# wns349/tensorflow-yolo

Measured on AMD Instinct MI355X. Metric: images/sec at 1/2/4/8 MI355X + post-NMS box-set match vs CPU ref, higher is better.
Workload: dtype f16; 1 GPU; v3-608-b32-fp16; network=v3, batch_per_gpu=32, global_batch=32, weights=seeded synthetic Darknet stream (random-init), streams=1

## Files before the change

### tensorflow-yolo_amd/csrc/conv_tap.hip

```cpp
#include "conv_common.h"
#include "conv_tiles.h"
#include <cstdio>
#include <type_traits>
#include <utility>

#ifndef YOLO_TAP_ASM_MFMA
#define YOLO_TAP_ASM_MFMA 1
#endif
#ifndef YOLO_TAP_W_FIRST
#define YOLO_TAP_W_FIRST 1
#endif
#ifndef YOLO_TAP_AH_ALL
#define YOLO_TAP_AH_ALL 1
#endif
#ifndef YOLO_TAP_PIL_RECOMPUTE
#define YOLO_TAP_PIL_RECOMPUTE 0
#endif
#ifndef YOLO_TAP_PIL
#define YOLO_TAP_PIL 1
#endif
#ifndef YOLO_TAP_DBG
#define YOLO_TAP_DBG 0
#endif
#ifndef YOLO_TAP_RECOMPUTE_ADDR
#define YOLO_TAP_RECOMPUTE_ADDR 1
#endif
#ifndef YOLO_TAP_LATE_FROM
#define YOLO_TAP_LATE_FROM 4
#endif
#ifndef YOLO_TAP_STAGGER
#define YOLO_TAP_STAGGER 1
#endif

namespace yolo {

namespace {

typedef __attribute__((address_space(3))) void tap_lds_void;

__device__ __forceinline__ void tap_dma16(__amdgpu_buffer_rsrc_t rsrc, unsigned char *lds_dst, uint32_t voff, uint32_t soff) {
#if defined(__HIP_DEVICE_COMPILE__)
    __builtin_amdgcn_raw_ptr_buffer_load_lds(rsrc, (tap_lds_void *)lds_dst, 16, voff, soff, 0, 0);
#else
    (void)rsrc; (void)lds_dst; (void)voff; (void)soff;
#endif
}

template <typename T>
__device__ __forceinline__ void tap_mfma(float4v &acc, const uint4v &a, const uint4v &b) {
#if YOLO_TAP_ASM_MFMA && defined(__HIP_DEVICE_COMPILE__)
    if constexpr (sizeof(T) == 2) {
        asm volatile("v_mfma_f32_16x16x32_f16 %0, %1, %2, %0" : "+v"(acc) : "v"(a), "v"(b));
        return;
    }
#endif
    acc = mma_chunk<T>(a, b, acc);
}

template <int TM, int TP>
__device__ __forceinline__ void tap_mfma_drain(float4v (&acc)[TM][TP]) {
#if YOLO_TAP_ASM_MFMA && defined(__HIP_DEVICE_COMPILE__)
    asm volatile("s_nop 15\n\ts_nop 15" : "+v"(acc[0][0]));
#pragma unroll
    for (int a = 0; a < TM; ++a)
#pragma unroll
        for (int b = 0; b < TP; ++b) asm volatile("" : "+v"(acc[a][b]));
#endif
}

template <int N>
__device__ __forceinline__ void tap_wait_vm() {
    asm volatile("s_waitcnt vmcnt(%0)" ::"n"(N) : "memory");
}

__device__ __forceinline__ int tap_swz_w(int r) { return (0x78 >> (2 * ((r >> 2) & 3))) & 3; }

constexpr int kTapStreamBiasFloats = 512;

}

template <bool F32, int WM, int WN, int TM, int TP, int PRG, int OCC, int MODE, bool SPLITK, bool FAST = false, bool FUSE2 = false>
__global__ void __launch_bounds__(WM * WN * 64, OCC) conv3x3_tap_kernel(const ConvParams p) {
    typedef typename std::conditional<F32, float, _Float16>::type T;
    constexpr bool TWO_D = MODE == 2 || MODE == 3;
    constexpr bool S2 = MODE == 4;
    constexpr int PADQ = TWO_D ? 2 : 1;
    constexpr int NW = WM * WN;
    constexpr int S = 3;
    constexpr bool STAG = YOLO_TAP_STAGGER != 0 && !F32 && !SPLITK && TM % 2 == 0 && NW == 8 && MODE == 4 && OCC == 4;
    constexpr int TMH = TM / 2;
    constexpr bool PIL = YOLO_TAP_PIL != 0 && MODE == 1 && !F32;
    constexpr int PL = (PRG * 16) / TP;
    constexpr int ROWB = 64;
    constexpr int NA = WM * TM * 16;
    constexpr int NB = WN * TP * 16;
    constexpr int JA_TOT = NA / 16;
    constexpr int JA = (JA_TOT + NW - 1) / NW;
    constexpr int PW = (TWO_D && OCC >= 6) ? 18 : 24;
    constexpr int FROW = TWO_D ? PW : 16;
    constexpr int JP = (PRG + NW - 1) / NW;
    constexpr int CH = 4 * TM;
    constexpr int A_BYTES = NA * ROWB;
    constexpr int P_BYTES = PRG * 1024;
    static_assert(NW == 8, "eight waves");
    static_assert(JA_TOT % NW == 0 || JA_TOT < NW, "weight tile must split evenly over the waves (or be smaller than them)");
    static_assert(!TWO_D || PRG * 16 >= (NB / 16 + 2) * PW, "patch buffer too small for the 2-D tile");
    if constexpr (F32 && (TP > 2 || OCC >= 6)) return;
    if constexpr (SPLITK && !(WM == 2 && WN == 4 && TM == 4 && (TP == 2 || ((TP == 4 || TP == 3) && !F32)) && MODE == 1)) return;
    if constexpr (MODE == 3 && (TP % 2 != 0 || SPLITK)) return;
    static_assert(!FAST || (!F32 && !SPLITK && MODE != 3), "the lean epilogue: fp16, whole K, plain output");
    static_assert(!S2 || JA_TOT % NW == 0, "stride 2: every wave carries weights");
    if constexpr (S2 && (F32 || SPLITK)) return;
    static_assert(!FUSE2 || (FAST && WM == 2 && WN == 4 && TM == 4 && TP == 4), "back-to-back 1x1: the 128 x 256 tiles (eight waves)");
    constexpr int LDS_BYTES = FUSE2 && kFuse2LdsBytes > S * A_BYTES + 2 * P_BYTES ? kFuse2LdsBytes : S * A_BYTES + 2 * P_BYTES;
    __shared__ __attribute__((aligned(16))) unsigned char smem[LDS_BYTES];
    unsigned char *const smemP = smem + S * A_BYTES;

    const int tid = threadIdx.x;
#ifdef YOLO_EXPERIMENT
    const unsigned long long t_start = p.trace ? wall_clock64() : 0ull;
    const unsigned long long c_start = p.trace ? (unsigned long long)clock64() : 0ull;
    if ((p.dbg & 64) && ((__builtin_amdgcn_s_getreg(0xF804) >> 16) & 1u)) __builtin_amdgcn_s_setprio(3);
    if ((p.dbg >> 8) > 0 && ((__builtin_amdgcn_s_getreg(0xF804) >> 16) & 1u)) {
        const unsigned long long until = wall_clock64() + (unsigned long long)(p.dbg >> 8) * 25ull;
        while (wall_clock64() < until) __builtin_amdgcn_s_sleep(4);
    }
#endif
    const int lane = tid & 63;
    const int wave = __builtin_amdgcn_readfirstlane(tid >> 6);
    const int wm = wave / WN, wn = wave % WN;

    const int bid = xcd_remap(blockIdx.x, p.n_blocks);
    const int mt = (int)fdiv((uint32_t)bid, p.dtiles_n);
    const int nt = bid - mt * p.n_tiles_n;
    const int n0 = nt * NA;
    const int q0 = mt * p.q_stride;
    const bool has_a = JA_TOT % NW == 0 || wave < JA_TOT;

    const __amdgpu_buffer_rsrc_t rs_in = __builtin_amdgcn_make_buffer_rsrc(const_cast<void *>(p.in), 0, p.in_bytes, 0x00020000);
    const __amdgpu_buffer_rsrc_t rs_w = __builtin_amdgcn_make_buffer_rsrc(const_cast<void *>(p.wgt), 0, p.wgt_bytes, 0x00020000);

    const int lrow = lane >> 2;
    uint32_t a_off[JA];
#pragma unroll
    for (int j = 0; j < JA; ++j) {
        const int r = (j * NW + wave) * 16 + lrow;
        const int ws = r / (TM * 16), R = r % (TM * 16);
        const int tm = R >> 4, g4 = (R >> 2) & 3, jj = R & 3;
        const int ch = ws * (TM * 16) + g4 * CH + 4 * tm + jj;
        a_off[j] = (uint32_t)(n0 + ch) * p.wrow_bytes + (uint32_t)(((lane & 3) ^ tap_swz_w(lrow)) << 4);
    }
    const int c_begin = SPLITK ? (int)blockIdx.y * p.kunits : 0;
    const int C = SPLITK ? ((c_begin + p.kunits < (p.cin_chunks >> 2)) ? c_begin + p.kunits : (p.cin_chunks >> 2)) : (p.cin_chunks >> 2);
    const int KT = 9 * C;
    auto issue_weights = [&](int tap, int c, int slot) {
        const uint32_t ka = (uint32_t)(tap * p.cin_chunks + 4 * c) * 16;
        if (has_a) {
#pragma unroll
            for (int j = 0; j < JA; ++j) tap_dma16(rs_w, smem + slot * A_BYTES + (j * NW + wave) * 1024, a_off[j], ka);
        }
    };
    constexpr bool W_FIRST = YOLO_TAP_W_FIRST != 0 && YOLO_TAP_PIL != 0 && MODE == 1 && !F32;
    if constexpr (W_FIRST) {
        issue_weights(0, c_begin, 0);
        issue_weights(1, c_begin, 1);
        __builtin_amdgcn_sched_barrier(0);
    }
    constexpr int JP_FULL = PRG - (JP - 1) * NW;
    const bool jp_full = wave < JP_FULL;
    uint32_t b_off[JP];
    const uint32_t csw_p = (uint32_t)(((lane & 3) ^ (((lrow >> 2) & 1) << 1)) << 4);
    int t2_n = 0, t2_y0 = 0, t2_x0 = 0;
    if (TWO_D) {
        t2_n = (int)fdiv((uint32_t)mt, p.dqHW);
        const int r = mt - t2_n * p.qHW;
        const int ty = (int)fdiv((uint32_t)r, p.dqW);
        t2_y0 = ty * (NB / 16);
        t2_x0 = (r - ty * p.qW) * 16;
    }
#pragma unroll
    for (int j = 0; j < JP; ++j) {
        const int g = j * NW + wave;
        bool ok;
        int n, y, x;
        if (TWO_D) {
            const int R = g * 16 + lrow;
            const int pr = R / PW, pc = R - pr * PW;
            n = t2_n; y = t2_y0 - 1 + pr; x = t2_x0 - 1 + pc;
            ok = g < PRG && pc < 18 && pr < NB / 16 + 2 && t2_n * p.HoWo < p.M && (unsigned)y < (unsigned)p.H && (unsigned)x < (unsigned)p.W;
        } else {
            int Rp = g * 16 + lrow;
            bool in_planes = true;
            if constexpr (PIL) {
                const int plane = Rp / PL, idx = Rp - plane * PL;
                in_planes = plane < TP;
                Rp = idx * TP + plane;
            }
            const int q = q0 - (p.qW + 1) + Rp;
            ok = g < PRG && in_planes && q >= 0 && q < p.Mq;
            const int qq = ok ? q : 0;
            n = (int)fdiv((uint32_t)qq, p.dqHW);
            const int r = qq - n * p.qHW;
            y = (int)fdiv((uint32_t)r, p.dqW);
            x = r - y * p.qW;
            if (S2) { ok = ok && x < p.Wo && y < p.Ho; y *= 2; x *= 2; }
            else ok = ok && x < p.W && y < p.H;
        }
        const long long e = (long long)n * p.in_img_stride + ((long long)y * p.W + x) * p.in_ld + p.in_coff;
        b_off[j] = ok ? (uint32_t)(e * (long long)sizeof(T)) + csw_p : YOLO_INVALID_OFF;
    }

    auto issue_patch = [&](int c, int buf, uint32_t plane_off = 0u) {
        const uint32_t koff = (uint32_t)c * ROWB + plane_off;
#pragma unroll
        for (int j = 0; j < JP; ++j)
            if (j + 1 < JP || jp_full) tap_dma16(rs_in, smemP + buf * P_BYTES + (j * NW + wave) * 1024, b_off[j], koff);
    };

    float4v acc[TM][TP];
    float4v acc2[F32 ? TM : 1][F32 ? TP : 1];
    const int fr = lane & 15, fq = lane >> 4;
    auto init_acc = [&]() {
        if constexpr (SPLITK) {
            if ((TP != 2 || p.pair) && blockIdx.y == 0) {
                conv_init_acc_bias<TM, TP>(p, acc, n0 + wm * (TM * 16) + fq * CH);
            } else {
#pragma unroll
                for (int a = 0; a < TM; ++a)
#pragma unroll
                    for (int b = 0; b < TP; ++b) acc[a][b] = float4v{0.f, 0.f, 0.f, 0.f};
            }
        } else {
            conv_init_acc_bias<TM, TP>(p, acc, n0 + wm * (TM * 16) + fq * CH);
        }
    };
    if constexpr (!STAG) init_acc();
    if constexpr (F32) {
#pragma unroll
        for (int a = 0; a < TM; ++a)
#pragma unroll
            for (int b = 0; b < TP; ++b) acc2[F32 ? a : 0][F32 ? b : 0] = float4v{0.f, 0.f, 0.f, 0.f};
    }

    const int a_frag = (wm * TM * 16 + fr) * ROWB + (((fq ^ tap_swz_w(fr)) & 3) << 4);
    const int rb = wn * TP * FROW + fr;

    auto compute = [&](int slot, int buf, int shift) {
        const unsigned char *A = smem + slot * A_BYTES + a_frag;
        if constexpr (!TWO_D && YOLO_TAP_RECOMPUTE_ADDR && STAG) asm volatile("" : "+s"(shift));
        const int R = rb + shift;
        const unsigned char *B = smemP + buf * P_BYTES + (R << 6) + ((fq << 4) ^ ((R & 4) << 3));
        uint4v fa[TM], fb[TP];
        if constexpr ((YOLO_TAP_DBG & 64) != 0) {
#pragma unroll
            for (int a = 0; a < TM; ++a) asm volatile("" : "=v"(fa[a]));
#pragma unroll
            for (int b = 0; b < TP; ++b) asm volatile("" : "=v"(fb[b]));
        } else {
#pragma unroll
        for (int a = 0; a < TM; ++a) {
            if constexpr ((YOLO_TAP_DBG & 128) != 0) { if (a == TM - 1) { asm volatile("" : "=v"(fa[a])); continue; } }
            fa[a] = *reinterpret_cast<const uint4v *>(A + a * 16 * ROWB);
        }
#pragma unroll
        for (int b = 0; b < TP; ++b) {
            if constexpr ((YOLO_TAP_DBG & 128) != 0) { if (b == TP - 1) { asm volatile("" : "=v"(fb[b])); continue; } }
            if constexpr (TWO_D && (FROW & 7) != 0) {
                const int Rb = R + b * FROW;
                fb[b] = *reinterpret_cast<const uint4v *>(smemP + buf * P_BYTES + (Rb << 6) + ((fq << 4) ^ ((Rb & 4) << 3)));
            } else {
                fb[b] = *reinterpret_cast<const uint4v *>(B + b * FROW * ROWB);
            }
        }
        }
#pragma unroll
        for (int a = 0; a < TM; ++a)
#pragma unroll
            for (int b = 0; b < TP; ++b) tap_mfma<T>(acc[a][b], fa[a], fb[b]);
    };

    uint4v G[PIL ? TP : 1];
    auto g_ptr = [&](int buf, int u) {
        if constexpr (YOLO_TAP_PIL_RECOMPUTE != 0) asm volatile("" : "+s"(u));
        const int plane = (int)((unsigned)u % (unsigned)TP), idx0 = (int)((unsigned)u / (unsigned)TP);
        const int L = plane * PL + idx0 + fr;
        return smemP + buf * P_BYTES + (L << 6) + ((fq << 4) ^ ((L & 4) << 3));
    };
    auto compute_pil = [&](int slot, int buf, int kh, int kw, int nbuf, auto &&issue_dma) {
        if constexpr (PIL) {
            const unsigned char *A = smem + slot * A_BYTES + a_frag;
            const int u0 = kh * p.qW + wn * (TP * 16);
            constexpr int AH = YOLO_TAP_AH_ALL ? TM : (TM >= 4 ? TM / 2 : TM);
            uint4v fa[TM];
#pragma unroll
            for (int a0 = 0; a0 < TM; a0 += AH) {
#pragma unroll
                for (int a = a0; a < a0 + AH; ++a) fa[a] = *reinterpret_cast<const uint4v *>(A + a * 16 * ROWB);
                if (a0 == 0) issue_dma();
#pragma unroll
                for (int a = a0; a < a0 + AH; ++a)
#pragma unroll
                    for (int b = 0; b < TP; ++b) tap_mfma<T>(acc[a][b], fa[a], G[(b + kw) % TP]);
            }
            if (kw < 2) G[kw % TP] = *reinterpret_cast<const uint4v *>(g_ptr(buf, u0 + TP + kw));
            else {
                const int un = (kh < 2 ? (kh + 1) * p.qW : 0) + wn * (TP * 16);
#pragma unroll
                for (int b = 0; b < TP; ++b) G[b] = *reinterpret_cast<const uint4v *>(g_ptr(nbuf, un + b));
            }
        }
    };

    uint4v ha[STAG ? TMH : 1], hb[STAG ? TP : 1];
    auto late_finish = [&]() {
        if constexpr (STAG) {
#pragma unroll
            for (int a = 0; a < TMH; ++a)
#pragma unroll
                for (int b = 0; b < TP; ++b) tap_mfma<T>(acc[TMH + a][b], ha[a], hb[b]);
        }
    };
    auto compute_late = [&](int slot, int buf, int shift) {
        if constexpr (STAG) {
            late_finish();
            __builtin_amdgcn_sched_barrier(0);
            const unsigned char *A = smem + slot * A_BYTES + a_frag;
            if constexpr (!TWO_D && YOLO_TAP_RECOMPUTE_ADDR) asm volatile("" : "+s"(shift));
            const int R = rb + shift;
            const unsigned char *B = smemP + buf * P_BYTES + (R << 6) + ((fq << 4) ^ ((R & 4) << 3));
            uint4v fa[TMH];
#pragma unroll
            for (int a = 0; a < TMH; ++a) fa[a] = *reinterpret_cast<const uint4v *>(A + a * 16 * ROWB);
#pragma unroll
            for (int b = 0; b < TP; ++b) {
                if constexpr (TWO_D && (FROW & 7) != 0) {
                    const int Rb = R + b * FROW;
                    hb[b] = *reinterpret_cast<const uint4v *>(smemP + buf * P_BYTES + (Rb << 6) + ((fq << 4) ^ ((Rb & 4) << 3)));
                } else {
                    hb[b] = *reinterpret_cast<const uint4v *>(B + b * FROW * ROWB);
                }
            }
#pragma unroll
            for (int a = 0; a < TMH; ++a)
#pragma unroll
                for (int b = 0; b < TP; ++b) tap_mfma<T>(acc[a][b], fa[a], hb[b]);
            __builtin_amdgcn_sched_barrier(0);
#pragma unroll
            for (int a = 0; a < TMH; ++a) ha[a] = *reinterpret_cast<const uint4v *>(A + (TMH + a) * 16 * ROWB);
            asm volatile("s_waitcnt lgkmcnt(0)" ::: "memory");
        }
    };
    const bool late = STAG && wave >= YOLO_TAP_LATE_FROM;
#ifdef YOLO_EXPERIMENT
    const unsigned long long t_setup = p.trace ? wall_clock64() : 0ull;
#endif
    const uint32_t pl01 = S2 ? (uint32_t)p.in_ld * 2u : 0u, pl10 = S2 ? (uint32_t)(p.W * p.in_ld) * 2u : 0u;
    if constexpr (S2) {
        issue_patch(c_begin, 0, pl10 + pl01);
        issue_weights(0, c_begin, 0);
        issue_weights(2, c_begin, 1);
    } else if constexpr (W_FIRST) {
        issue_patch(c_begin, 0);
    } else {
        issue_patch(c_begin, 0);
        issue_weights(0, c_begin, 0);
        issue_weights(1, c_begin, 1);
    }
    auto run_slice_s2 = [&](int c, auto bufc, auto latec) {
        constexpr int X = decltype(bufc)::value, Y = X ^ 1;
        constexpr bool LATE = decltype(latec)::value;
        constexpr int kTapOf[9] = {0, 2, 4, 6, 8, 1, 7, 3, 5};
        constexpr int kBufOf[9] = {X, X, Y, X, X, Y, Y, X, X};
        constexpr int kShOf[9] = {0, 1, 3, 2, 3, 1, 3, 2, 3};
        const bool more = c + 1 < C;
#pragma unroll
        for (int s = 0; s < 9; ++s) {
            const bool last = !more && s == 8;
            const bool patch_prev = s == 1 || s == 4 || s == 6 || (s == 8 && more);
            if (last) tap_wait_vm<0>();
            else if (!patch_prev) tap_wait_vm<JA>();
            else if (jp_full) tap_wait_vm<JA + JP>();
            else tap_wait_vm<JA + JP - 1>();
            __builtin_amdgcn_sched_barrier(0);
            __builtin_amdgcn_s_barrier();
            {
                const int s2 = s + 2 < 9 ? s + 2 : s + 2 - 9;
                const int c2 = s + 2 < 9 ? c : c + 1;
                if (c2 < C) issue_weights(kTapOf[s2], c2, (s + 2) % S);
            }
            if (s == 0) issue_patch(c, Y, 0u);
            if (s == 3) issue_patch(c, Y, pl10);
            if (s == 5) issue_patch(c, X, pl01);
            if (s == 7 && more) issue_patch(c + 1, Y, pl10 + pl01);
            if constexpr (LATE) compute_late(s % S, kBufOf[s], ((kShOf[s] & 2) ? p.qW : 0) + (kShOf[s] & 1));
            else compute(s % S, kBufOf[s], ((kShOf[s] & 2) ? p.qW : 0) + (kShOf[s] & 1));
        }
    };

    auto run_slice = [&](int c, auto bufc, auto latec) {
        constexpr int buf = decltype(bufc)::value;
        constexpr bool LATE = decltype(latec)::value;
        const bool more = c + 1 < C;
#pragma unroll
        for (int tap = 0; tap < 9; ++tap) {
            const bool last = !more && tap == 8;
            const bool with_patch = more && (tap == 1 || tap == 2);
            if constexpr ((YOLO_TAP_DBG & 32) != 0) { if (last) tap_wait_vm<0>(); } else
            if (last) tap_wait_vm<0>();
            else if (has_a) {
                if (!with_patch) tap_wait_vm<JA>();
                else if (jp_full) tap_wait_vm<JA + JP>();
                else tap_wait_vm<JA + JP - 1>();
            } else {
                if (!with_patch) tap_wait_vm<0>();
                else if (jp_full) tap_wait_vm<JP>();
                else tap_wait_vm<JP - 1>();
            }
            __builtin_amdgcn_sched_barrier(0);
            if constexpr (!((YOLO_TAP_DBG & 16) != 0 || ((YOLO_TAP_DBG & 8) != 0 && tap % 3 != 0))) __builtin_amdgcn_s_barrier();
            auto issue_dma = [&]() {
                {
                    const int t2 = tap + 2 < 9 ? tap + 2 : tap + 2 - 9;
                    const int c2 = tap + 2 < 9 ? c : c + 1;
                    if (c2 < C) issue_weights(t2, c2, (tap + 2) % S);
                }
                if (tap == 0 && more) issue_patch(c + 1, buf ^ 1);
            };
            const int kh = tap / 3, kw = tap - 3 * kh;
            if constexpr (PIL && !LATE) compute_pil(tap % S, buf, kh, kw, tap == 8 ? buf ^ 1 : buf, issue_dma);
            else {
                issue_dma();
                if constexpr (LATE) compute_late(tap % S, buf, TWO_D ? kh * PW + kw : kh * p.qW + kw);
                else compute(tap % S, buf, TWO_D ? kh * PW + kw : kh * p.qW + kw);
            }
        }
    };
    if constexpr (PIL) {
        if (has_a && !W_FIRST) tap_wait_vm<2 * JA>(); else tap_wait_vm<0>();
        __builtin_amdgcn_s_barrier();
#pragma unroll
        for (int b = 0; b < TP; ++b) G[b] = *reinterpret_cast<const uint4v *>(g_ptr(0, wn * (TP * 16) + b));
        __builtin_amdgcn_sched_barrier(0);
    }
    auto run_all = [&](auto latec) {
        if constexpr (STAG) init_acc();
        if constexpr (decltype(latec)::value) {
#pragma unroll
            for (int a = 0; a < TMH; ++a) ha[a] = uint4v{0u, 0u, 0u, 0u};
#pragma unroll
            for (int b = 0; b < TP; ++b) hb[b] = uint4v{0u, 0u, 0u, 0u};
        }
        for (int c = c_begin; c < C; c += 2) {
            if constexpr (S2) {
                run_slice_s2(c, std::integral_constant<int, 0>(), latec);
                if (c + 1 < C) run_slice_s2(c + 1, std::integral_constant<int, 1>(), latec);
            } else {
                run_slice(c, std::integral_constant<int, 0>(), latec);
                if (c + 1 < C) run_slice(c + 1, std::integral_constant<int, 1>(), latec);
            }
            if constexpr (F32) flush_acc<TM, TP>(acc, acc2);
        }
    };
    if constexpr (STAG) {
        if (late) {
            run_all(std::true_type());
            late_finish();
        } else {
            run_all(std::false_type());
        }
    } else {
        run_all(std::false_type());
    }
    if constexpr (!F32) tap_mfma_drain<TM, TP>(acc);
    if constexpr (F32) {
#pragma unroll
        for (int a = 0; a < TM; ++a)
#pragma unroll
            for (int b = 0; b < TP; ++b) acc[a][b] = acc2[a][b];
    }
    (void)KT;
#ifdef YOLO_EXPERIMENT
    const unsigned long long t_loop = p.trace ? wall_clock64() : 0ull;
#endif
    if constexpr (SPLITK) {
        if constexpr (TP == 2) {
            if (!p.pair) {
                conv_store_partial<TM, TP, PADQ, PIL>(p, acc, n0 + wm * (TM * 16) + fq * CH, q0 + wn * (TP * 16), fr, (int)blockIdx.y);
                return;
            }
        }
        constexpr uint32_t SLAB = (uint32_t)NA * NB * 4;
        const __amdgpu_buffer_rsrc_t rs_part = __builtin_amdgcn_make_buffer_rsrc(p.part, 0, p.part_bytes, 0x00020000);
        const uint32_t nsplit = gridDim.y;
        const uint32_t mine = ((uint32_t)blockIdx.x * nsplit + blockIdx.y) * SLAB, other = ((uint32_t)blockIdx.x * nsplit + (1u - blockIdx.y)) * SLAB;
        typedef __attribute__((__vector_size__(4 * sizeof(unsigned int)))) unsigned int u4;
#pragma unroll
        for (int a = 0; a < TM; ++a)
#pragma unroll
            for (int b = 0; b < TP; ++b)
                __builtin_amdgcn_raw_buffer_store_b128(__builtin_bit_cast(u4, acc[a][b]), rs_part,
                                                       mine + (uint32_t)((((wave * TM + a) * TP + b) * 64 + lane) * 16), 0, 16 );
        asm volatile("s_waitcnt vmcnt(0)" ::: "memory");
        __syncthreads();
        int *const flag = reinterpret_cast<int *>(smem);
        if (tid == 0) {
            int *const ticket = p.pair_cnt + (size_t)blockIdx.x * kCandCountStride;
            const int t = __hip_atomic_fetch_add(ticket, 1, __ATOMIC_RELAXED, __HIP_MEMORY_SCOPE_AGENT);
            if (t == (int)nsplit - 1) {
                __hip_atomic_store(ticket, 0, __ATOMIC_RELAXED, __HIP_MEMORY_SCOPE_AGENT);
                __builtin_amdgcn_fence(__ATOMIC_ACQUIRE, "agent");
                asm volatile("s_waitcnt vmcnt(0)" ::: "memory");
            }
            *flag = t;
        }
        __syncthreads();
        if (*flag != (int)nsplit - 1) return;
        if (nsplit > 2) {
#pragma unroll
            for (int a = 0; a < TM; ++a)
#pragma unroll
                for (int b = 0; b < TP; ++b) acc[a][b] = float4v{0.f, 0.f, 0.f, 0.f};
            for (uint32_t sp = 0; sp < nsplit; ++sp) {
                const uint32_t base = ((uint32_t)blockIdx.x * nsplit + sp) * SLAB;
#pragma unroll
                for (int a = 0; a < TM; ++a) {
                    u4 v[TP];
#pragma unroll
                    for (int b = 0; b < TP; ++b)
                        v[b] = __builtin_amdgcn_raw_buffer_load_b128(rs_part, base + (uint32_t)((((wave * TM + a) * TP + b) * 64 + lane) * 16), 0, 16 );
#pragma unroll
                    for (int b = 0; b < TP; ++b) acc[a][b] += __builtin_bit_cast(float4v, v[b]);
                }
            }
            conv_epilogue<T, TM, TP, PADQ, true, PIL>(p, acc, n0 + wm * (TM * 16) + fq * CH, q0 + wn * (TP * 16), fr);
            return;
        }
#pragma unroll
        for (int a = 0; a < TM; ++a) {
            u4 v[TP];
#pragma unroll
            for (int b = 0; b < TP; ++b)
                v[b] = __builtin_amdgcn_raw_buffer_load_b128(rs_part, other + (uint32_t)((((wave * TM + a) * TP + b) * 64 + lane) * 16), 0, 16 );
#pragma unroll
            for (int b = 0; b < TP; ++b) acc[a][b] += __builtin_bit_cast(float4v, v[b]);
            __builtin_amdgcn_sched_barrier(0);
        }
        conv_epilogue<T, TM, TP, PADQ, true, PIL>(p, acc, n0 + wm * (TM * 16) + fq * CH, q0 + wn * (TP * 16), fr);
        return;
    } else {
        if constexpr (MODE == 3) conv_epilogue_pool2<T, TM, TP>(p, acc, n0 + wm * (TM * 16) + fq * CH, q0 + wn * (TP * 16), fr);
        else if constexpr (FUSE2) {
            static_assert(!FUSE2 || 2 * LDS_BYTES <= 163840, "two workgroups per CU");
            if constexpr (S2) conv_epilogue_fused_1x1<PADQ, false>(p, acc, q0, wm, wn, wave, lane, smem);
            else conv_epilogue_fused_1x1<PADQ, true>(p, acc, q0, wm, wn, wave, lane, smem);
        }
        else if constexpr (FAST) conv_epilogue_fast<TM, TP, PADQ, PIL>(p, acc, n0 + wm * (TM * 16) + fq * CH, q0 + wn * (TP * 16), fr);
        else conv_epilogue<T, TM, TP, PADQ, true, PIL>(p, acc, n0 + wm * (TM * 16) + fq * CH, q0 + wn * (TP * 16), fr);
    }
#ifdef YOLO_EXPERIMENT
    if (p.trace && tid == 0) {
        asm volatile("s_waitcnt vmcnt(0)" ::: "memory");
        unsigned long long *r = p.trace + (size_t)blockIdx.x * 8;
        r[0] = t_start; r[1] = t_setup; r[2] = t_loop; r[3] = wall_clock64();
        r[4] = __builtin_amdgcn_s_getreg(0xF804);
        r[5] = __builtin_amdgcn_s_getreg(0xF814);
        r[6] = (unsigned long long)bid;
        r[7] = (unsigned long long)clock64() - c_start;
    }
#endif
}

template <int WM, int WN, int TM, int TP, int PRG, int OCC, int MODE>
__global__ void __launch_bounds__(512, OCC) conv3x3_tap_stream_kernel(const ConvParams p) {
    typedef _Float16 T;
    constexpr int NW = 8, S = 3, ROWB = 64;
    constexpr int NA = WM * TM * 16;
    constexpr int NB = WN * TP * 16;
    constexpr int JA_TOT = NA / 16;
    constexpr int JA = (JA_TOT + NW - 1) / NW;
    constexpr int PW = 24;
    constexpr int FROW = MODE == 2 ? PW : 16;
    constexpr int JP = (PRG + NW - 1) / NW;
    constexpr int CH = 4 * TM;
    constexpr int EPC = 8;
    constexpr int NQ = CH / EPC;
    constexpr int NST = TP * NQ;
    constexpr int A_BYTES = NA * ROWB;
    constexpr int P_BYTES = PRG * 1024;
    constexpr int BIAS_FLOATS = kTapStreamBiasFloats;
    static_assert(WM * WN == NW && (JA_TOT % NW == 0 || JA_TOT < NW), "tile / wave mapping");
    __shared__ __attribute__((aligned(16))) unsigned char smem[S * A_BYTES + 2 * P_BYTES + BIAS_FLOATS * 4];
    unsigned char *const smemP = smem + S * A_BYTES;
    float *const sbias = reinterpret_cast<float *>(smem + S * A_BYTES + 2 * P_BYTES);

    const int tid = threadIdx.x;
    const int lane = tid & 63;
    const int wave = __builtin_amdgcn_readfirstlane(tid >> 6);
    const int wm = wave / WN, wn = wave % WN;
    const bool has_a = JA_TOT % NW == 0 || wave < JA_TOT;
    const int fr = lane & 15, fq = lane >> 4;

    const __amdgpu_buffer_rsrc_t rs_in = __builtin_amdgcn_make_buffer_rsrc(const_cast<void *>(p.in), 0, p.in_bytes, 0x00020000);
    const __amdgpu_buffer_rsrc_t rs_w = __builtin_amdgcn_make_buffer_rsrc(const_cast<void *>(p.wgt), 0, p.wgt_bytes, 0x00020000);
    const __amdgpu_buffer_rsrc_t rs_out = __builtin_amdgcn_make_buffer_rsrc(p.out, 0, p.out_bytes, 0x00020000);
    const __amdgpu_buffer_rsrc_t rs_res = __builtin_amdgcn_make_buffer_rsrc(const_cast<void *>(p.res ? p.res : p.out), 0, p.res ? p.res_bytes : 0u, 0x00020000);

    for (int i = tid; i < p.cout_pad && i < BIAS_FLOATS; i += 512) sbias[i] = p.bias[i];

    const int lrow = lane >> 2;
    uint32_t a_off[JA];
#pragma unroll
    for (int j = 0; j < JA; ++j) {
        const int r = (j * NW + wave) * 16 + lrow;
        const int ws = r / (TM * 16), R = r % (TM * 16);
        const int tm = R >> 4, g4 = (R >> 2) & 3, jj = R & 3;
        const int ch = ws * (TM * 16) + g4 * CH + 4 * tm + jj;
        a_off[j] = (uint32_t)ch * p.wrow_bytes + (uint32_t)(((lane & 3) ^ tap_swz_w(lrow)) << 4);
    }
    constexpr int JP_FULL = PRG - (JP - 1) * NW;
    const bool jp_full = wave < JP_FULL;
    const uint32_t csw_p = (uint32_t)(((lane & 3) ^ (((lrow >> 2) & 1) << 1)) << 4);
    uint32_t b_off[JP];
    auto geometry = [&](int bid, int &q0, int &n0) __attribute__((always_inline)) {
        const int mt = (int)fdiv((uint32_t)bid, p.dtiles_n);
        n0 = (bid - mt * p.n_tiles_n) * NA;
        q0 = mt * NB;
        int t2_n = 0, t2_y0 = 0, t2_x0 = 0;
        if (MODE == 2) {
            t2_n = (int)fdiv((uint32_t)mt, p.dqHW);
            const int r = mt - t2_n * p.qHW;
            const int ty = (int)fdiv((uint32_t)r, p.dqW);
            t2_y0 = ty * (NB / 16);
            t2_x0 = (r - ty * p.qW) * 16;
        }
#pragma unroll
        for (int j = 0; j < JP; ++j) {
            const int g = j * NW + wave;
            bool ok;
            int n, y, x;
            if (MODE == 2) {
                const int R = g * 16 + lrow;
                const int pr = R / PW, pc = R - pr * PW;
                n = t2_n; y = t2_y0 - 1 + pr; x = t2_x0 - 1 + pc;
                ok = g < PRG && pc < 18 && pr < NB / 16 + 2 && t2_n * p.HoWo < p.M && (unsigned)y < (unsigned)p.H && (unsigned)x < (unsigned)p.W;
            } else {
                const int q = q0 - (p.qW + 1) + g * 16 + lrow;
                ok = g < PRG && q >= 0 && q < p.Mq;
                const int qq = ok ? q : 0;
                n = (int)fdiv((uint32_t)qq, p.dqHW);
                const int r = qq - n * p.qHW;
                y = (int)fdiv((uint32_t)r, p.dqW);
                x = r - y * p.qW;
                ok = ok && x < p.W && y < p.H;
            }
            const long long e = (long long)n * p.in_img_stride + ((long long)y * p.W + x) * p.in_ld + p.in_coff;
            b_off[j] = ok ? (uint32_t)(e * 2) + csw_p : YOLO_INVALID_OFF;
        }
    };

    const int C = p.cin_chunks >> 2;
    auto issue_patch = [&](int c, int buf) __attribute__((always_inline)) {
        const uint32_t koff = (uint32_t)c * ROWB;
#pragma unroll
        for (int j = 0; j < JP; ++j)
            if (j + 1 < JP || jp_full) tap_dma16(rs_in, smemP + buf * P_BYTES + (j * NW + wave) * 1024, b_off[j], koff);
    };
    auto issue_weights = [&](int tap, int c, int n0, int slot) __attribute__((always_inline)) {
        const uint32_t ka = (uint32_t)(tap * p.cin_chunks + 4 * c) * 16 + (uint32_t)n0 * p.wrow_bytes;
        if (has_a) {
#pragma unroll
            for (int j = 0; j < JA; ++j) tap_dma16(rs_w, smem + slot * A_BYTES + (j * NW + wave) * 1024, a_off[j], ka);
        }
    };

    float4v acc[TM][TP];
    const int a_frag = (wm * TM * 16 + fr) * ROWB + (((fq ^ tap_swz_w(fr)) & 3) << 4);
    const int rb = wn * TP * FROW + fr;
    const int c_lane = wm * (TM * 16) + fq * CH;
    auto compute = [&](int slot, int buf, int shift) __attribute__((always_inline)) {
        const unsigned char *A = smem + slot * A_BYTES + a_frag;
        const int R = rb + shift;
        const unsigned char *B = smemP + buf * P_BYTES + (R << 6) + ((fq << 4) ^ ((R & 4) << 3));
        uint4v fa[TM], fb[TP];
#pragma unroll
        for (int a = 0; a < TM; ++a) fa[a] = *reinterpret_cast<const uint4v *>(A + a * 16 * ROWB);
#pragma unroll
        for (int b = 0; b < TP; ++b) fb[b] = *reinterpret_cast<const uint4v *>(B + b * FROW * ROWB);
#pragma unroll
        for (int a = 0; a < TM; ++a)
#pragma unroll
            for (int b = 0; b < TP; ++b) tap_mfma<T>(acc[a][b], fa[a], fb[b]);
    };
    auto epilogue = [&](int q0, int n0) __attribute__((always_inline)) {
        constexpr int DEPTH = TP > 2 ? 2 : TP;
        const int cbase = n0 + c_lane;
        const bool c_ok = cbase < p.Cout;
        uint32_t ooff[DEPTH];
        uint4v rv[DEPTH][NQ];
        auto request = [&](int b, int slot) __attribute__((always_inline)) {
            int n, rem, oy, ox;
            const bool ok = conv_decode_pixel<MODE>(p, q0 + wn * (TP * 16) + b * 16 + fr, n, rem, oy, ox) && c_ok;
            const long long o = ((long long)n * p.out_img_stride + (long long)rem * p.out_ld + cbase) * 2;
            ooff[slot] = ok ? (uint32_t)o : YOLO_INVALID_OFF;
            if (p.has_res) {
                const long long ro = ((long long)n * p.res_img_stride + (long long)rem * p.res_ld + cbase) * 2;
                const uint32_t roff = ok ? (uint32_t)ro : YOLO_INVALID_OFF;
#pragma unroll
                for (int q = 0; q < NQ; ++q)
                    rv[slot][q] = __builtin_bit_cast(uint4v, __builtin_amdgcn_raw_buffer_load_b128(rs_res, roff, q * 16, 0));
            }
        };
#pragma unroll
        for (int b = 0; b < DEPTH; ++b) request(b, b);
#pragma unroll
        for (int b = 0; b < TP; ++b) {
            const int slot = b % DEPTH;
#pragma unroll
            for (int q = 0; q < NQ; ++q) {
                T t[EPC], r[EPC];
                if (p.has_res) __builtin_memcpy(r, &rv[slot][q], 16);
#pragma unroll
                for (int e = 0; e < EPC; ++e) {
                    const int i = q * EPC + e;
                    float x = acc[i >> 2][b][i & 3];
                    x = p.leaky ? fmaxf(0.1f * x, x) : x;
                    if (p.has_res) x += (float)r[e];
                    t[e] = (T)x;
                }
                uint4v u;
                __builtin_memcpy(&u, t, 16);
                __builtin_amdgcn_raw_buffer_store_b128(__builtin_bit_cast(__attribute__((__vector_size__(4 * sizeof(unsigned int)))) unsigned int, u), rs_out, ooff[slot], q * 16, 0);
            }
            if (b + DEPTH < TP) {
                __builtin_amdgcn_sched_barrier(0);
                request(b + DEPTH, slot);
            }
        }
    };
    auto init_acc = [&](int n0, bool from_lds) __attribute__((always_inline)) {
#pragma unroll
        for (int a = 0; a < TM; ++a) {
            const float4v bv = from_lds ? *reinterpret_cast<const float4v *>(sbias + n0 + c_lane + 4 * a)
                                        : *reinterpret_cast<const float4v *>(p.bias + n0 + c_lane + 4 * a);
#pragma unroll
            for (int b = 0; b < TP; ++b) acc[a][b] = bv;
        }
    };

    int it = blockIdx.x;
    int q0_cur, n0_cur, q0_nxt = 0, n0_nxt = 0;
    geometry(xcd_remap(it, p.n_blocks), q0_cur, n0_cur);
    init_acc(n0_cur, false);
    issue_patch(0, 0);
    issue_weights(0, 0, n0_cur, 0);
    issue_weights(1, 0, n0_cur, 1);
    int c = 0;
    bool after_epi = false;
    bool done = false;

    auto run_item = [&](auto bufc) __attribute__((always_inline)) {
        constexpr int buf = decltype(bufc)::value;
        const bool last_c = c + 1 == C;
        const int it_n = last_c ? it + (int)gridDim.x : it;
        const bool more = !last_c || it_n < p.n_blocks;
        const int c_n = last_c ? 0 : c + 1;
        if (!last_c) { n0_nxt = n0_cur; q0_nxt = q0_cur; }
#pragma unroll
        for (int tap = 0; tap < 9; ++tap) {
            const bool last = !more && tap == 8;
            const bool with_patch = more && (tap == 1 || tap == 2);
            const bool st = after_epi && tap < 2;
            if (last) tap_wait_vm<0>();
            else if (has_a) {
                if (!with_patch) { if (st) tap_wait_vm<JA + NST>(); else tap_wait_vm<JA>(); }
                else if (jp_full) { if (st) tap_wait_vm<JA + JP + NST>(); else tap_wait_vm<JA + JP>(); }
                else { if (st) tap_wait_vm<JA + JP - 1 + NST>(); else tap_wait_vm<JA + JP - 1>(); }
            } else {
                if (!with_patch) { if (st) tap_wait_vm<NST>(); else tap_wait_vm<0>(); }
                else if (jp_full) { if (st) tap_wait_vm<JP + NST>(); else tap_wait_vm<JP>(); }
                else { if (st) tap_wait_vm<JP - 1 + NST>(); else tap_wait_vm<JP - 1>(); }
            }
            __builtin_amdgcn_sched_barrier(0);
            __builtin_amdgcn_s_barrier();
            if (tap == 0 && more) {
                if (last_c) geometry(xcd_remap(it_n, p.n_blocks), q0_nxt, n0_nxt);
            }
            {
                if (tap + 2 < 9) issue_weights(tap + 2, c, n0_cur, (tap + 2) % S);
                else if (more) issue_weights(tap + 2 - 9, c_n, n0_nxt, (tap + 2) % S);
            }
            if (tap == 0 && more) issue_patch(c_n, buf ^ 1);
            const int kh = tap / 3, kw = tap - 3 * kh;
            compute(tap % S, buf, MODE == 2 ? kh * PW + kw : kh * p.qW + kw);
        }
        after_epi = false;
        if (last_c) {
            tap_mfma_drain<TM, TP>(acc);
            epilogue(q0_cur, n0_cur);
            if (!more) { done = true; return; }
            it = it_n; q0_cur = q0_nxt; n0_cur = n0_nxt;
            init_acc(n0_cur, true);
            after_epi = true;
        }
        c = c_n;
    };
    for (;;) {
        run_item(std::integral_constant<int, 0>());
        if (done) break;
        run_item(std::integral_constant<int, 1>());
        if (done) break;
    }
}

bool conv_tap_fits(const ConvTile &t, int W) {
    if (!t.is_tap()) return false;
    if (t.is2d()) return true;
    if (t.stride2()) {
        if (W & 1) return false;
        W >>= 1;
    }
    if (t.image_aligned() && (W * (W + 1) > t.nb() || W * (W + 1) * 5 < t.nb() * 4)) return false;
    if (t.stride2()) return t.nb() + W + 2 <= t.prg * 16;
    const int rows = YOLO_TAP_PIL ? t.prg * 16 / t.tp * t.tp : t.prg * 16;
    return t.nb() + 2 * W + 4 <= rows;
}

static bool tap_stream_ok(const ConvTile &t, const ConvParams &p) {
    if (!t.has(CAP_STREAM)) return false;
    if (p.f32 || p.out_f32 || p.ksplit > 1 || p.outmode != OUT_NORMAL || !p.vec_out || (p.has_res && (!p.vec_res || !p.res_bytes)) || !p.out_bytes) return false;
    return p.Cout % 16 == 0 && (p.Cout + 127) / 128 * 128 <= kTapStreamBiasFloats;
}

static bool tap_lean(const ConvTile &t, const ConvParams &p) {
    static const bool no_fast_epi = getenv("YOLO_NO_FAST_EPI") != nullptr;
    return (!no_fast_epi || p.fuse2) && conv_fast_epilogue_ok(p) && (!t.has(CAP_NO_LEAN) || p.fuse2);
}

static ConvForm tap_form(const ConvTile &t, const ConvParams &p) {
    if (!t.is_tap() || (p.f32 && !t.f32_ok())) return FORM_INVALID;
    if (p.stream && tap_stream_ok(t, p)) return FORM_STREAM;
    if (p.ksplit > 1) return (p.pair ? t.split_occ != 0 : t.has(CAP_SPLITK)) ? FORM_SPLITK : FORM_INVALID;
    if (p.outmode == OUT_POOL2) return t.has(CAP_POOL) ? FORM_POOL : FORM_INVALID;
    if (p.fuse2) return t.has(CAP_FUSE2) && tap_lean(t, p) ? FORM_FUSED : FORM_INVALID;
    return !p.f32 && tap_lean(t, p) ? FORM_LEAN : FORM_GENERIC;
}

struct TapInst { bool f32; int occ, mode; bool splitk, fast, fuse2; };
static constexpr TapInst tap_inst(const ConvTile &t, ConvForm f, bool f32) {
    return {f32, f == FORM_SPLITK ? t.split_occ : t.occ, f == FORM_POOL ? 3 : t.mode, f == FORM_SPLITK, f == FORM_LEAN || f == FORM_FUSED, f == FORM_FUSED};
}

std::string conv_tap_symbol(const ConvTile &t, const ConvParams &p) {
    const ConvForm f = tap_form(t, p);
    if (f == FORM_INVALID) return "";
    char b[192];
    auto tf = [](bool v) { return v ? "true" : "false"; };
    const TapInst i = tap_inst(t, f, p.f32 != 0);
    if (f == FORM_STREAM) snprintf(b, sizeof b, "void yolo::conv3x3_tap_stream_kernel<%d, %d, %d, %d, %d, %d, %d>(yolo::ConvParams)", t.wm, t.wn, t.tm, t.tp, t.prg, t.occ, t.mode);
    else snprintf(b, sizeof b, "void yolo::conv3x3_tap_kernel<%s, %d, %d, %d, %d, %d, %d, %d, %s, %s, %s>(yolo::ConvParams)", tf(i.f32), t.wm, t.wn, t.tm, t.tp, t.prg,
                  i.occ, i.mode, tf(i.splitk), tf(i.fast), tf(i.fuse2));
    return b;
}

template <int ID, ConvForm F, bool F32>
static hipError_t launch_tap_inst(const ConvParams &p, dim3 grid, hipStream_t s) {
    constexpr ConvTile t = kTiles[ID];
    constexpr TapInst i = tap_inst(t, F, F32);
    hipLaunchKernelGGL((conv3x3_tap_kernel<i.f32, t.wm, t.wn, t.tm, t.tp, t.prg, i.occ, i.mode, i.splitk, i.fast, i.fuse2>), grid, dim3(512), 0, s, p);
    return hipGetLastError();
}
template <int ID, ConvForm F, bool HAS_F32>
static hipError_t launch_tap_dtype(const ConvParams &p, dim3 grid, hipStream_t s) {
    if constexpr (HAS_F32) if (p.f32) return launch_tap_inst<ID, F, true>(p, grid, s);
    return launch_tap_inst<ID, F, false>(p, grid, s);
}

template <int ID>
static hipError_t launch_tap_tile(ConvForm f, const ConvParams &p0, dim3 grid, hipStream_t s) {
    constexpr ConvTile t = kTiles[ID];
    if constexpr (t.is_tap()) {
        switch (f) {
        case FORM_GENERIC: return launch_tap_dtype<ID, FORM_GENERIC, true>(p0, grid, s);
        case FORM_LEAN: return launch_tap_inst<ID, FORM_LEAN, false>(p0, grid, s);
        case FORM_SPLITK: if constexpr (t.split_occ != 0) return launch_tap_dtype<ID, FORM_SPLITK, t.f32_ok()>(p0, grid, s); break;
        case FORM_POOL: if constexpr (t.has(CAP_POOL)) return launch_tap_dtype<ID, FORM_POOL, t.f32_ok()>(p0, grid, s); break;
        case FORM_FUSED: if constexpr (t.has(CAP_FUSE2)) return launch_tap_inst<ID, FORM_FUSED, false>(p0, grid, s); break;
        case FORM_STREAM:
            if constexpr (t.has(CAP_STREAM)) {
                ConvParams p = p0;
                p.cout_pad = (p.Cout + 127) / 128 * 128;
                constexpr int slots = kTapStreamCUs * t.per_cu();
                static_assert(slots == kTapStreamGrid, "yolo_launch_caps reports kTapStreamGrid");
                hipLaunchKernelGGL((conv3x3_tap_stream_kernel<t.wm, t.wn, t.tm, t.tp, t.prg, t.occ, t.mode>), dim3((unsigned)(p.n_blocks < slots ? p.n_blocks : slots)), dim3(512), 0, s, p);
                return hipGetLastError();
            }
            break;
        default: break;
        }
    }
    return hipErrorInvalidValue;
}
template <int... ID>
static hipError_t launch_tap_by_id(int id, ConvForm f, const ConvParams &p, dim3 grid, hipStream_t s, std::integer_sequence<int, ID...>) {
    hipError_t e = hipErrorInvalidValue;
    (void)((id == ID && ((e = launch_tap_tile<ID>(f, p, grid, s)), true)) || ...);
    return e;
}

hipError_t launch_conv_tap(const ConvParams &p0, int tile, hipStream_t s) {
    if (tile < 0 || tile >= kNumTiles) return hipErrorInvalidValue;
    const ConvTile &t = conv_tile(tile);
    ConvParams p = p0;
    p.fast_epi = tap_lean(t, p) ? 1 : 0;
    const bool s2 = t.stride2();
    if (p.ksize != 3 || p.stride != (s2 ? 2 : 1) || p.pad != 1 || (p.cin_chunks & 3) || !conv_tap_fits(t, p.W) || (p.f32 && !t.f32_ok()))
        return hipErrorInvalidValue;
    if (s2 ? ((p.H & 1) || (p.W & 1) || p.Ho * 2 != p.H || p.Wo * 2 != p.W || p.f32 || p.ksplit > 1 || (p.fuse2 && !t.has(CAP_FUSE2)) || p.outmode == OUT_POOL2 || p.qW != p.Wo + 1)
           : (p.Ho != p.H || p.Wo != p.W))
        return hipErrorInvalidValue;
    if (t.image_aligned() ? (p.q_stride != p.qHW || p.Ho * (p.Wo + 1) > t.nb()) : (!t.is2d() && p.q_stride != t.nb()))
        return hipErrorInvalidValue;
    if (p.outmode == OUT_POOL2 && (!t.has(CAP_POOL) || (p.H & 1) || (p.W & 1) || p.has_res || p.ksplit > 1 || !p.vec_out || p.Cout % 16))
        return hipErrorInvalidValue;
    const ConvForm f = tap_form(t, p);
    if (f == FORM_SPLITK) {
        if (!p.part || p.kunits < 1 || (long long)p.ksplit * p.kunits < (p.cin_chunks >> 2)) return hipErrorInvalidValue;
        if (p.pair && (p.ksplit < 2 || (p.ksplit > 2 && !t.has(CAP_SPLITK)) || !p.pair_cnt || p.n_blocks > 512 ||
                       (unsigned long long)p.n_blocks * (unsigned long long)p.ksplit * 128ull * t.nb() * 4ull > p.part_bytes))
            return hipErrorInvalidValue;
    }
    if (f == FORM_FUSED && (t.has(CAP_FUSE2_RES) != (p.has_res != 0) || p.n_tiles_n != 1 || p.Cout != 128 || !p.w2 || !p.b2 || !p.out2 || !p.out2_bytes))
        return hipErrorInvalidValue;
    const dim3 grid((unsigned)p.n_blocks, (unsigned)(p.ksplit > 1 ? p.ksplit : 1));
    return launch_tap_by_id(tile, f, p, grid, s, std::make_integer_sequence<int, kNumTiles>());
}

}
```

Measured before the change: 6256 images/sec.

## Add weight-resident 3x3 tap-stream path for single-chunk, single-N-tile convs

For MODE 2 tap-stream convs where the whole input-channel depth fits in one chunk and Cout fits in one N tile, all nine tap weight slices are loaded into LDS once per workgroup. After that the kernel loops over spatial tiles, double-buffering only a compact 18-wide input patch. The goal is to stop re-streaming weights through the 3-stage ring on every tile and to cut per-tap synchronisation. It uses more LDS, which could lower occupancy, and it adds a new code path with its own patch addressing and swizzle.

```diff
diff --git a/tensorflow-yolo_amd/csrc/conv_tap.hip b/tensorflow-yolo_amd/csrc/conv_tap.hip
--- a/tensorflow-yolo_amd/csrc/conv_tap.hip
+++ b/tensorflow-yolo_amd/csrc/conv_tap.hip
@@ -589,9 +589,19 @@
     constexpr int P_BYTES = PRG * 1024;
     constexpr int BIAS_FLOATS = kTapStreamBiasFloats;
     static_assert(WM * WN == NW && (JA_TOT % NW == 0 || JA_TOT < NW), "tile / wave mapping");
-    __shared__ __attribute__((aligned(16))) unsigned char smem[S * A_BYTES + 2 * P_BYTES + BIAS_FLOATS * 4];
+    constexpr int RPW = 18;
+    constexpr int RPRG = ((NB / 16 + 2) * RPW + 15) / 16;
+    constexpr int RJP = (RPRG + NW - 1) / NW;
+    constexpr int RP_BYTES = RPRG * 1024;
+    constexpr int RING_LDS = S * A_BYTES + 2 * P_BYTES + BIAS_FLOATS * 4;
+    constexpr int RES_LDS = MODE == 2 ? 9 * A_BYTES + 2 * RP_BYTES + NA * 4 : 0;
+    static_assert(MODE != 2 || OCC != 4 || 2 * RES_LDS <= 163840, "the resident form keeps two workgroups per CU");
+    static_assert(RJP <= JP, "the resident form's patch offsets live in b_off");
+    __shared__ __attribute__((aligned(16))) unsigned char smem[RES_LDS > RING_LDS ? RES_LDS : RING_LDS];
+    const bool resident = MODE == 2 && p.stream == 2;
     unsigned char *const smemP = smem + S * A_BYTES;
-    float *const sbias = reinterpret_cast<float *>(smem + S * A_BYTES + 2 * P_BYTES);
+    unsigned char *const smemQ = smem + 9 * A_BYTES;
+    float *const sbias = reinterpret_cast<float *>(smem + (resident ? 9 * A_BYTES + 2 * RP_BYTES : S * A_BYTES + 2 * P_BYTES));
 
     const int tid = threadIdx.x;
     const int lane = tid & 63;
@@ -605,7 +615,7 @@
     const __amdgpu_buffer_rsrc_t rs_out = __builtin_amdgcn_make_buffer_rsrc(p.out, 0, p.out_bytes, 0x00020000);
     const __amdgpu_buffer_rsrc_t rs_res = __builtin_amdgcn_make_buffer_rsrc(const_cast<void *>(p.res ? p.res : p.out), 0, p.res ? p.res_bytes : 0u, 0x00020000);
 
-    for (int i = tid; i < p.cout_pad && i < BIAS_FLOATS; i += 512) sbias[i] = p.bias[i];
+    for (int i = tid; i < p.cout_pad && i < (resident ? NA : BIAS_FLOATS); i += 512) sbias[i] = p.bias[i];
 
     const int lrow = lane >> 2;
     uint32_t a_off[JA];
@@ -621,7 +631,9 @@
     const bool jp_full = wave < JP_FULL;
     const uint32_t csw_p = (uint32_t)(((lane & 3) ^ (((lrow >> 2) & 1) << 1)) << 4);
     uint32_t b_off[JP];
-    auto geometry = [&](int bid, int &q0, int &n0) __attribute__((always_inline)) {
+    auto geometry = [&](auto resc, int bid, int &q0, int &n0) __attribute__((always_inline)) {
+        constexpr bool RES = decltype(resc)::value;
+        constexpr int pw = RES ? RPW : PW, prg = RES ? RPRG : PRG, jp = RES ? RJP : JP;
         const int mt = (int)fdiv((uint32_t)bid, p.dtiles_n);
         n0 = (bid - mt * p.n_tiles_n) * NA;
         q0 = mt * NB;
@@ -634,18 +646,18 @@
             t2_x0 = (r - ty * p.qW) * 16;
         }
 #pragma unroll
-        for (int j = 0; j < JP; ++j) {
+        for (int j = 0; j < jp; ++j) {
             const int g = j * NW + wave;
             bool ok;
             int n, y, x;
             if (MODE == 2) {
                 const int R = g * 16 + lrow;
-                const int pr = R / PW, pc = R - pr * PW;
+                const int pr = R / pw, pc = R - pr * pw;
                 n = t2_n; y = t2_y0 - 1 + pr; x = t2_x0 - 1 + pc;
-                ok = g < PRG && pc < 18 && pr < NB / 16 + 2 && t2_n * p.HoWo < p.M && (unsigned)y < (unsigned)p.H && (unsigned)x < (unsigned)p.W;
+                ok = g < prg && pc < 18 && pr < NB / 16 + 2 && t2_n * p.HoWo < p.M && (unsigned)y < (unsigned)p.H && (unsigned)x < (unsigned)p.W;
             } else {
                 const int q = q0 - (p.qW + 1) + g * 16 + lrow;
-                ok = g < PRG && q >= 0 && q < p.Mq;
+                ok = g < prg && q >= 0 && q < p.Mq;
                 const int qq = ok ? q : 0;
                 n = (int)fdiv((uint32_t)qq, p.dqHW);
                 const int r = qq - n * p.qHW;
@@ -747,9 +759,75 @@
         }
     };
 
+    if constexpr (MODE == 2) if (resident) {
+        constexpr int RJP_FULL = RPRG - (RJP - 1) * NW;
+        const bool rjp_full = wave < RJP_FULL;
+        auto issue_patch_r = [&](int buf) __attribute__((always_inline)) {
+#pragma unroll
+            for (int j = 0; j < RJP; ++j)
+                if (j + 1 < RJP || rjp_full) tap_dma16(rs_in, smemQ + buf * RP_BYTES + (j * NW + wave) * 1024, b_off[j], 0u);
+        };
+        const int rbr = wn * TP * RPW + fr;
+        auto compute_r = [&](int tap, int buf) __attribute__((always_inline)) {
+            const unsigned char *A = smem + tap * A_BYTES + a_frag;
+            const int kh = tap / 3, kw = tap - 3 * kh;
+            uint4v fa[TM], fb[TP];
+#pragma unroll
+            for (int a = 0; a < TM; ++a) fa[a] = *reinterpret_cast<const uint4v *>(A + a * 16 * ROWB);
+#pragma unroll
+            for (int b = 0; b < TP; ++b) {
+                const int Rb = rbr + (kh + b) * RPW + kw;
+                fb[b] = *reinterpret_cast<const uint4v *>(smemQ + buf * RP_BYTES + (Rb << 6) + ((fq << 4) ^ ((Rb & 4) << 3)));
+            }
+#pragma unroll
+            for (int a = 0; a < TM; ++a)
+#pragma unroll
+                for (int b = 0; b < TP; ++b) tap_mfma<T>(acc[a][b], fa[a], fb[b]);
+        };
+        int it = blockIdx.x;
+        int q0_cur, q0_nxt = 0, n0_r;
+        geometry(std::true_type(), xcd_remap(it, p.n_blocks), q0_cur, n0_r);
+        init_acc(0, false);
+        if (has_a) {
+#pragma unroll
+            for (int tap = 0; tap < 9; ++tap)
+#pragma unroll
+                for (int j = 0; j < JA; ++j) tap_dma16(rs_w, smem + tap * A_BYTES + (j * NW + wave) * 1024, a_off[j], (uint32_t)(tap * p.cin_chunks) * 16);
+        }
+        issue_patch_r(0);
+        bool first = true, done = false;
+        auto run_tile = [&](auto bufc) __attribute__((always_inline)) {
+            constexpr int buf = decltype(bufc)::value;
+            const int it_n = it + (int)gridDim.x;
+            const bool more = it_n < p.n_blocks;
+            if (first) tap_wait_vm<0>(); else tap_wait_vm<NST>();
+            __builtin_amdgcn_sched_barrier(0);
+            __builtin_amdgcn_s_barrier();
+            if (more) {
+                geometry(std::true_type(), xcd_remap(it_n, p.n_blocks), q0_nxt, n0_r);
+                issue_patch_r(buf ^ 1);
+            }
+#pragma unroll
+            for (int tap = 0; tap < 9; ++tap) compute_r(tap, buf);
+            tap_mfma_drain<TM, TP>(acc);
+            epilogue(q0_cur, 0);
+            if (!more) { done = true; return; }
+            it = it_n; q0_cur = q0_nxt;
+            init_acc(0, true);
+            first = false;
+        };
+        for (;;) {
+            run_tile(std::integral_constant<int, 0>());
+            if (done) break;
+            run_tile(std::integral_constant<int, 1>());
+            if (done) break;
+        }
+        return;
+    }
+
     int it = blockIdx.x;
     int q0_cur, n0_cur, q0_nxt = 0, n0_nxt = 0;
-    geometry(xcd_remap(it, p.n_blocks), q0_cur, n0_cur);
+    geometry(std::false_type(), xcd_remap(it, p.n_blocks), q0_cur, n0_cur);
     init_acc(n0_cur, false);
     issue_patch(0, 0);
     issue_weights(0, 0, n0_cur, 0);
@@ -783,7 +861,7 @@
             __builtin_amdgcn_sched_barrier(0);
             __builtin_amdgcn_s_barrier();
             if (tap == 0 && more) {
-                if (last_c) geometry(xcd_remap(it_n, p.n_blocks), q0_nxt, n0_nxt);
+                if (last_c) geometry(std::false_type(), xcd_remap(it_n, p.n_blocks), q0_nxt, n0_nxt);
             }
             {
                 if (tap + 2 < 9) issue_weights(tap + 2, c, n0_cur, (tap + 2) % S);
@@ -829,6 +907,11 @@
     if (!t.has(CAP_STREAM)) return false;
     if (p.f32 || p.out_f32 || p.ksplit > 1 || p.outmode != OUT_NORMAL || !p.vec_out || (p.has_res && (!p.vec_res || !p.res_bytes)) || !p.out_bytes) return false;
     return p.Cout % 16 == 0 && (p.Cout + 127) / 128 * 128 <= kTapStreamBiasFloats;
+}
+
+static bool tap_resident(const ConvParams &p) {
+    static const bool no_resident = getenv("YOLO_NO_TAP_RESIDENT") != nullptr;
+    return !no_resident && (p.cin_chunks >> 2) == 1 && p.n_tiles_n == 1;
 }
 
 static bool tap_lean(const ConvTile &t, const ConvParams &p) {
@@ -889,6 +972,7 @@
             if constexpr (t.has(CAP_STREAM)) {
                 ConvParams p = p0;
                 p.cout_pad = (p.Cout + 127) / 128 * 128;
+                if (t.mode == 2 && tap_resident(p)) p.stream = 2;
                 constexpr int slots = kTapStreamCUs * t.per_cu();
                 static_assert(slots == kTapStreamGrid, "yolo_launch_caps reports kTapStreamGrid");
                 hipLaunchKernelGGL((conv3x3_tap_stream_kernel<t.wm, t.wn, t.tm, t.tp, t.prg, t.occ, t.mode>), dim3((unsigned)(p.n_blocks < slots ? p.n_blocks : slots)), dim3(512), 0, s, p);
```

Result: no change. 6253 images/sec (-0.1%).
